# QueensGambit/CrazyAra

Hardware: AMD Instinct MI355X
Metric: nn_evals_per_sec (higher is better)
Workload: dtype f16x3; 1 GPU; crazyhouse RISEv2 19-block (34x8x8 planes -> 5184 policy + value), batch=256, inputs resident in HBM, random-init seeded weights; batch=256, parallelism=replicas x1, precision=float16x3

## Files before the change

### crazyara_amd/csrc/nn/precision.cpp

```cpp
#include <cstdlib>
#include <stdexcept>

#include "rise_net.h"

namespace cra {

namespace {
constexpr bool kX3ValueHeadOneLaunch = true;
}

RiseNet::DevSwitches::DevSwitches() {
    if (const char* e = getenv("CRA_X3_CONV_DEV")) conv_dev = atoi(e);
    device_graph = getenv("CRA_DEVICE_GRAPH") != nullptr;
    lane_graph = getenv("CRA_LANE_GRAPH") != nullptr;
    lane_no_graph = getenv("CRA_LANE_NO_GRAPH") != nullptr;
    predict_copy = getenv("CRA_PREDICT_COPY") != nullptr;
    predict_zero_copy = getenv("CRA_PREDICT_ZERO_COPY") != nullptr;
    if (const char* e = getenv("CRA_LANE_LAUNCHES")) lane_launches = e[0];
    lane_sync = getenv("CRA_LANE_SYNC") != nullptr;
    if (const char* e = getenv("CRA_X3_TOWER")) x3_symmetric = e[0] == 's';
    if (const char* e = getenv("CRA_X3_SPLIT_DEV")) x3_split_dev = atoi(e);
    no_small_path = getenv("CRA_NO_SMALL_PATH") != nullptr;
    if (const char* e = getenv("CRA_SMALL_BATCH_CONV_SPLIT")) small_conv_split = atoi(e);
    tower_trace = getenv("CRA_TOWER_TRACE") != nullptr;
    x3_value_one_launch = kX3ValueHeadOneLaunch;
    if (const char* e = getenv("CRA_X3_VALUE_HEAD")) x3_value_one_launch = e[0] == 'o';
    value_head_debug = getenv("CRA_VALUE_HEAD_DEBUG") != nullptr;
    if (const char* e = getenv("CRA_VALUE_HEAD_LDS_PAD")) value_head_lds_pad = atoi(e);
    if (const char* e = getenv("CRA_VALUE_HEAD_VARIANT")) value_head_variant = atoi(e);
    x3_no_head_chain = getenv("CRA_X3_NO_HEAD_CHAIN") != nullptr;
    x3_no_tail = getenv("CRA_X3_NO_TAIL") != nullptr;
    x3_no_quad = getenv("CRA_X3_NO_QUAD") != nullptr;
    small_batch_heads_apart = getenv("CRA_SMALL_BATCH_HEADS_APART") != nullptr;
}

Precision parse_precision(const std::string& precision) {
    Precision v;
    std::string prec = precision;
    auto strip = [&](const std::string& tag) {
        if (prec.size() <= tag.size() || prec.compare(prec.size() - tag.size(), tag.size(), tag) != 0) return false;
        prec.resize(prec.size() - tag.size());
        return true;
    };
    if (strip("-3k")) v.one_launch = false;
    if (strip("-8w")) v.thin_waves = true;
    if (strip("-1wg")) v.board_split = false;
    if (strip("-1b")) v.boards_per_wg = 1;
    else if (strip("-2b")) v.boards_per_wg = 2;
// ... 32 lines not shown
```

### crazyara_amd/csrc/nn/rise_net.h

```cpp
#pragma once
#include <hip/hip_runtime.h>
#include <memory>
#include <string>
#include <utility>
#include <vector>

#include "board_net.h"
#include "netfile.h"

namespace cra {

uint8_t float_to_e4m3(float v);
uint8_t float_to_e5m2(float v);

struct Precision {
    enum class Mode { Float32, Float16, Float16x3, Float16p8, Fp8, Int8 };
    Mode mode = Mode::Float16;
    bool fused = true;
    bool tower = true;
    bool one_launch = true;
    bool thin_waves = false;
    bool board_split = true;
    bool wblock = false;
    bool wnet = false;
// ... 96 lines not shown
        char lane_launches = 0;
        bool lane_sync = false;
        bool x3_symmetric = false;
        int x3_split_dev = 0;
        bool no_small_path = false;
        int small_conv_split = 2;
        bool tower_trace = false;
        bool x3_value_one_launch;
        bool value_head_debug = false;
        int value_head_lds_pad = -1;
        int value_head_variant = 0;
        bool x3_no_head_chain = false;
        bool x3_no_tail = false;
        bool x3_no_quad = false;
        bool small_batch_heads_apart = false;
        DevSwitches();
    } dev_;
    float* value_head_dbg_ = nullptr;

    std::string model_file_path_;
    Precision prec_;
    std::vector<std::pair<float, float>> int8_calib_;
    static constexpr int kBoardSplitMaxBatch = 64;
    std::unique_ptr<RiseNet> small_;
    bool owns_stream_ = true;
    int stream_slot_ = -1;
    std::string precision_arg_;
    int cu_count_ = 256;
    int launches_ = 0;
    hipGraph_t graph_ = nullptr;
// ... 12 lines not shown
```

### crazyara_amd/csrc/nn/rise_net.hip

```cpp
#include "rise_net.h"

#include <cmath>
#include <cstdio>
#include <cstring>
#include <fstream>
#include <algorithm>

#include "net_streams.h"
#include "onnx_import.h"
#include "rise_net_impl.h"
#include "../chess/planes_host.h"

namespace cra {

RiseNet::RiseNet(const std::string& model_path, int device_id, int batch_size, const std::string& precision, const RiseNet* parent)
    : BoardNet(device_id), impl_(new Impl) {
    if (batch_size <= 0) throw std::invalid_argument("batch size must be positive");
    precision_arg_ = precision;
    prec_ = parse_precision(precision);
    design_.batch = batch_size;

    std::string dir, file;
    auto ends_with = [&](const char* ext) { const size_t n = strlen(ext); return model_path.size() > n && model_path.compare(model_path.size() - n, n, ext) == 0; };
    if (ends_with(".cranet") || ends_with(".onnx")) {
// ... 60 lines not shown
    const int B = n > 0 ? n : design_.batch;
    const Op& op = im.ops[i];
    auto boards = [&](ConvArgs c) {
        if (n > 0 && c.batch == design_.batch && !c.out_rows_f32) c.batch = n;
        return c;
    };
    const float* planes = io ? io->planes : d_planes_;
    float* value = io ? io->value : d_value_;
    float* probs = io ? io->probs : d_probs_;
    float* aux = (io && d_aux_) ? (io->aux ? io->aux : d_aux_) : d_aux_;
    switch (op.kind) {
        case OpKind::PlanesToAct:
            launch_planes_to_act<T>(op.x == d_planes_ ? planes : static_cast<const float*>(op.x), static_cast<T*>(op.y), B, op.C, im.cin_pad, s);
            break;
        case OpKind::Conv:
            if (prec_.x3() && dev_.conv_dev >= 0) {
                ConvArgs c = boards(op.conv);
                c.dev = dev_.conv_dev;
                if (op.from_planes) c.planes = planes;
                if (op.fused_softmax) { c.softmax_out = probs; if (!keep_logits_) c.out = nullptr; }
                launch_conv_gemm_x3(c, s);
            } else if (prec_.x3() && op.from_planes) {
                ConvArgs c = boards(op.conv);
                c.planes = planes;
                launch_conv_gemm_x3(c, s);
            } else if (prec_.x3() && op.fused_softmax) {
                ConvArgs c = boards(op.conv);
                c.softmax_out = probs;
                if (!keep_logits_) c.out = nullptr;
                launch_conv_gemm_x3(c, s);
            } else if (prec_.x3()) launch_conv_gemm_x3(boards(op.conv), s);
// ... 152 lines not shown
        case OpKind::BlockX3Split: return "block_x3_split";
        case OpKind::X3SplitFinish: return "x3_split_finish";
        case OpKind::HeadsSmall: return "heads_small";
        case OpKind::Attention: return "attention";
        case OpKind::BlockX3W: return "block_x3w";
        case OpKind::NtbX3W: return "ntb_x3w";
        case OpKind::TowerX3W: return "tower_x3w";
        case OpKind::BlockX3WSplit: return "block_x3w_split";
        case OpKind::X3WSplitFinish: return "x3w_split_finish";
    }
    return "?";
}

const char* RiseNet::op_kernel(int i) const {
    const Op& op = impl_->ops.at(i);
    return op.kind == OpKind::TowerX3 ? tower_x3_kernel_name(op.tx) : op_name(i);
}

void RiseNet::time_ops(int iters, float* ms) {
    HIP_CHECK(hipSetDevice(device_));
    hipEvent_t e0, e1;
    HIP_CHECK(hipEventCreate(&e0));
    HIP_CHECK(hipEventCreate(&e1));
    const int n = int(impl_->ops.size());
    for (int it = 0; it < iters; ++it)
        for (int i = 0; i < n; ++i) {
            HIP_CHECK(hipEventRecord(e0, stream_));
            ForwardCall call;
            if (prec_.fp16()) launch_op<half_t>(i, stream_, call); else launch_op<float>(i, stream_, call);
            HIP_CHECK(hipEventRecord(e1, stream_));
// ... 453 lines not shown
```

### crazyara_amd/csrc/nn/rise_net_build.hip

```cpp
#include <algorithm>
#include <cmath>
#include <cstring>
#include <type_traits>

#include "../chess/planes_host.h"
#include "pack.h"
#include "rise_net_impl.h"

namespace cra {

namespace {
enum class Family {
    Tower,
    X3Tower,
    X3Split,
    Fused,
    WBlock,
    WSplit,
    WTower,
    Layers,
    Transformer,
    WNtb
};
struct BlockPlan {
// ... 50 lines not shown
    void add_se(Op op, bool consumer_fused);
    void stem();
    void dense_tower();
    void dense_layer_blocks();
    void bottleneck_blocks();
    void transformer_block(size_t i);
    void transformer_block_x3w(const NtbFold& n);
    void flush_tower();
    void flush_x3_run();
    void wsplit_finish();
    void flush_wrun();
    void one_launch_head();
    void policy_head();
    void softmax();
    void value_head();
    void merge_heads_small();
    void merge_forward();
};

template <typename T> void RiseNet::Builder<T>::read_model() {
    B = net.design_.batch;
    cin = int(nf.num("nb_input_channels"));
    C = int(nf.num("channels", 256));
    const int cop_init = int(nf.num("channels_operating_init"));
    const int cexp = int(nf.num("channel_expansion"));
    cv = int(nf.num("channels_value_head", 8));
    fc = int(nf.num("value_fc_size", 256));
    cp = int(nf.num("channels_policy_head"));
    wdl = nf.num("use_wdl") != 0 && nf.num("use_plys_to_end") != 0;
    std::vector<std::string> kernels = nf.list("kernels");
// ... 837 lines not shown
    im.ops.push_back(op);
}

template <typename T> void RiseNet::Builder<T>::merge_heads_small() {
    std::vector<Op>& ops = im.ops;
    if (x3_split && ops.size() >= 2 && ops.back().kind == OpKind::ValueHead && ops[ops.size() - 2].kind == OpKind::Conv &&
        ops[ops.size() - 2].fused_softmax && heads_small_fits(ops[ops.size() - 2].conv, ops.back().vh) && !dev.small_batch_heads_apart) {
        Op vh = ops.back();
        ops.pop_back();
        Op& op = ops.back();
        op.kind = OpKind::HeadsSmall;
        op.vh = vh.vh;
    }
}

template <typename T> void RiseNet::Builder<T>::merge_forward() {
    std::vector<Op>& ops = im.ops;
    if (prec.one_launch && ops.size() == 3 && ops[0].kind == OpKind::Stem && ops[1].kind == OpKind::Tower && ops[2].kind == OpKind::Head &&
        ops[1].tw.gate_in == nullptr && ops[1].tw.pool_out == nullptr) {
        Op op;
        op.kind = OpKind::Forward;
        op.st = ops[0].st;
        op.tw = ops[1].tw;
        op.hd = ops[2].hd;
        ops.assign(1, op);
        init_forward_kernel_attributes();
    }
}

template <typename T> void RiseNet::build(const NetFile& nf) {
// ... 6 lines not shown
    if (prec_.wnet && b.wblock_ops == 0 && b.wntb_ops == 0)
        throw std::runtime_error(std::string(prec_.wtower ? "`-wtower`" : "`-wnet`") + " runs the mobile-bottleneck and transformer blocks of 128 / 192 / 224-channel nets in one launch each: no block of this model qualifies (" +
                                 std::to_string(b.C) + " channels, " + (b.dense_blocks ? "dense residual blocks" : "mobile-bottleneck blocks") +
                                 "); use the precision without the suffix");
    if (prec_.wblock && !prec_.wnet && b.wblock_ops == 0)
        throw std::runtime_error("`-wblock` runs the mobile-bottleneck blocks of 128 / 192 / 224-channel nets in one launch each: no block of this model qualifies (" +
                                 std::to_string(b.C) + " channels, " + (b.dense_blocks ? "dense residual blocks" : "mobile-bottleneck blocks") +
                                 "); use the precision without the suffix");
    if (b.head_ok) {
        b.one_launch_head();
    } else {
        b.policy_head();
        b.softmax();
        b.value_head();
        b.merge_heads_small();
    }
    init_block_kernel_attributes<T>();
    init_x3_kernel_attributes();
    init_x3_wblock_kernel_attributes();
    init_x3_wsplit_kernel_attributes();
    init_x3_wtower_kernel_attributes();
    init_x3_wntb_kernel_attributes();
    init_tower_kernel_attributes();
    init_restower_kernel_attributes();
    init_head_kernel_attributes();
    b.merge_forward();
    design_.flops_per_position = 2.0 * b.macs;
    launches_ = int(impl_->ops.size());
}

template void RiseNet::build<half_t>(const NetFile& nf);
template void RiseNet::build<float>(const NetFile& nf);

// ... 2 lines not shown
```

### crazyara_amd/csrc/nn/rise_net_impl.h

```cpp
#pragma once
#include <stdexcept>
#include <string>
#include <utility>
#include <vector>

#include "kernels.h"
#include "rise_net.h"

namespace cra {

#define HIP_CHECK(expr)                                                                                      \
    do {                                                                                                     \
        hipError_t _e = (expr);                                                                              \
        if (_e != hipSuccess)                                                                                \
            throw std::runtime_error(std::string("HIP error ") + hipGetErrorString(_e) + " at " #expr);      \
    } while (0)

enum class OpKind { PlanesToAct, Conv, Depthwise, SE, ValueHead, Softmax, Block, ValueFinal, SEGate, Tower, Head, Stem, ResTower, Forward, TowerX3, BlockX3Split, X3SplitFinish, HeadsSmall, Attention, BlockX3W, NtbX3W, BlockX3WSplit, X3WSplitFinish, TowerX3W };

struct Op {
    OpKind kind;
    ConvArgs conv{};
    bool from_planes = false;
    bool fused_softmax = false;
    const void* x = nullptr;
    void* y = nullptr;
    const float *w0 = nullptr, *w1 = nullptr, *b0 = nullptr;
    int C = 0, ks = 0, se_kind = 0;
    ValueHeadArgs vh{};
    BlockArgs blk{};
    NtbArgs ntb{};
    ValueFinalArgs vf{};
    TowerArgs tw{};
    HeadArgs hd{};
    ResTowerArgs rt{};
    StemArgs st{};
    X3TowerArgs tx{};
    X3SplitArgs xs{};
    float* xs_y = nullptr;
// ... 44 lines not shown
```

### crazyara_amd/csrc/nn/x3.hip

```cpp
#include "kernels.h"
#include "device_utils.h"
#include "value_head_body.h"
#include "x3_device.h"

#include <algorithm>
#include <cstdlib>
#include <stdexcept>
#include <type_traits>

#ifndef X3_SGB_VALU
#define X3_SGB_VALU 10
#endif

namespace cra {

namespace {

typedef int i32x4_x3 __attribute__((ext_vector_type(4)));
typedef int i32x8_x3 __attribute__((ext_vector_type(8)));
__device__ __forceinline__ uint32_t x3_high_bytes(uint32_t p01, uint32_t p23) {
    return __builtin_amdgcn_perm(p23, p01, 0x07050301u);
}
__device__ __forceinline__ void split4_b8(const float (&v)[4], half4& hi, uint32_t& h8, uint32_t& l8) {
    uint32_t h[2], l[2];
// ... 9 lines not shown
    else asm volatile("" : "+v"(c) : "v"(a), "v"(b));
}
__device__ __forceinline__ i32x8_x3 x3_cat(const half8& lo16, const half8& hi16) {
    return __builtin_shufflevector(__builtin_bit_cast(i32x4_x3, lo16), __builtin_bit_cast(i32x4_x3, hi16), 0, 1, 2, 3, 4, 5, 6, 7);
}

__device__ __forceinline__ float fmac_shr1(float acc, float x, float w) { return fmaf(w, dpp_mov<DPP_ROW_SHR1>(x), acc); }
__device__ __forceinline__ float fmac_shl1(float acc, float x, float w) { return fmaf(w, dpp_mov<DPP_ROW_SHL1>(x), acc); }

__device__ __forceinline__ void mma_x3(const half8& ah, const half8& al, const half8& bh, const half8& bl, f32x4& c) {
    c = __builtin_amdgcn_mfma_f32_16x16x32_f16(al, bh, c, 0, 0, 0);
    c = __builtin_amdgcn_mfma_f32_16x16x32_f16(ah, bl, c, 0, 0, 0);
    c = __builtin_amdgcn_mfma_f32_16x16x32_f16(ah, bh, c, 0, 0, 0);
}

constexpr int X3_KC = 128;
constexpr int X3_ROWP = X3_KC + 8;

}

template <int MT, int NW>
__device__ __forceinline__ void conv_x3_finish(const ConvArgs& a, f32x4 (&acc)[MT][4], const bool (&active)[MT], char* smem, int b, int co_tile0, float acc_scale) {
    constexpr int NTHR = 64 * NW;
    const int tid = threadIdx.x;
    const int wave = tid >> 6, lane = tid & 63;
    const int l15 = lane & 15, lg = lane >> 4;
    if (a.softmax_out) __syncthreads();
#pragma unroll
    for (int m = 0; m < MT; ++m) {
        if (!active[m]) continue;
        const int co0 = (co_tile0 + m) * 16 + lg * 4;
        float bs[4];
#pragma unroll
        for (int r = 0; r < 4; ++r) bs[r] = a.bias[co0 + r];
#pragma unroll
        for (int t = 0; t < 4; ++t) {
            const int sq = t * 16 + l15;
            float v[4];
#pragma unroll
            for (int r = 0; r < 4; ++r) v[r] = fmaf(acc[m][t][r], acc_scale, bs[r]);
            if (a.relu == 2) {
#pragma unroll
                for (int r = 0; r < 4; ++r) v[r] = fmaxf(v[r], 0.f);
            }
            if (a.resid) {
                float rv[4];
                load4<float>(reinterpret_cast<const float*>(a.resid) + (size_t(b) * kSquares + sq) * a.cout_ld + co0, rv);
#pragma unroll
                for (int r = 0; r < 4; ++r) v[r] += rv[r];
            }
            if (a.relu == 1) {
#pragma unroll
                for (int r = 0; r < 4; ++r) v[r] = fmaxf(v[r], 0.f);
            }
            if (a.out_policy_f32) {
                float* o = reinterpret_cast<float*>(a.out) + size_t(b) * a.cout_real * kSquares;
                float* lds_logits = reinterpret_cast<float*>(smem);
#pragma unroll
                for (int r = 0; r < 4; ++r)
                    if (co0 + r < a.cout_real) {
                        if (a.out) o[(co0 + r) * kSquares + sq] = v[r];
                        if (a.softmax_out) lds_logits[(co0 + r) * kSquares + sq] = v[r];
                    }
            } else if (a.out_rows_f32) {
                const int row = b * kSquares + sq;
                if (row < a.rows_valid) {
                    float* o = reinterpret_cast<float*>(a.out) + size_t(row) * a.cout_real;
#pragma unroll
                    for (int r = 0; r < 4; ++r)
                        if (co0 + r < a.cout_real) o[co0 + r] = v[r];
                }
            } else if (a.out_flat) {
                float* o = reinterpret_cast<float*>(a.out) + size_t(b) * a.flat_pitch;
#pragma unroll
                for (int r = 0; r < 4; ++r)
                    if (co0 + r < a.cout_real) o[(co0 + r) * kSquares + sq] = v[r];
            } else {
                store4<float>(reinterpret_cast<float*>(a.out) + (size_t(b) * kSquares + sq) * a.cout_ld + co0, v);
            }
        }
    }
    if (a.softmax_out) {
        __syncthreads();
        const float* in = reinterpret_cast<const float*>(smem);
        float* red = reinterpret_cast<float*>(smem) + 8192;
        const int n = a.cout_real * kSquares;
        float* out = a.softmax_out + size_t(b) * n;
        float m = -INFINITY;
        for (int i = tid; i < n; i += NTHR) m = fmaxf(m, in[i]);
#pragma unroll
        for (int off = 32; off > 0; off >>= 1) m = fmaxf(m, __shfl_xor(m, off, 64));
        if (lane == 0) red[wave] = m;
        __syncthreads();
        m = red[0];
#pragma unroll
        for (int i = 1; i < NW; ++i) m = fmaxf(m, red[i]);
        float sum = 0.f;
        for (int i = tid; i < n; i += NTHR) sum += expf(in[i] - m);
#pragma unroll
        for (int off = 32; off > 0; off >>= 1) sum += __shfl_xor(sum, off, 64);
        __syncthreads();
        if (lane == 0) red[wave] = sum;
        __syncthreads();
        sum = red[0];
#pragma unroll
        for (int i = 1; i < NW; ++i) sum += red[i];
        const float c = m + logf(sum);
        for (int i = tid; i < n; i += NTHR) out[i] = expf(in[i] - c);
    }
}

template <int KS, int MT, int NW, int NS>
__device__ __forceinline__ void conv_gemm_x3_body(const ConvArgs& a, char* smem, const int bx, const int b) {
    half_t* xh = reinterpret_cast<half_t*>(smem);
    half_t* xl = xh + 65 * X3_ROWP;
    constexpr int ROWP = X3_ROWP, KC = X3_KC, NTHR = 64 * NW;

    const int tid = threadIdx.x;
    const int wave = tid >> 6, lane = tid & 63;
    const int l15 = lane & 15, lg = lane >> 4;
    const int co_tile0 = (bx * NW + wave) * MT;
    bool active[MT];
#pragma unroll
    for (int m = 0; m < MT; ++m) active[m] = (co_tile0 + m) * 16 < a.cout_pad;
    const int x_ld = a.x_ld ? a.x_ld : a.cin;
// ... 390 lines not shown
#pragma unroll
    for (int t = 0; t < 4; ++t) acc2[0][t] = f32x4{0.f, 0.f, 0.f, 0.f};
    ConvP8Window<1> W;
    if (active[0]) conv_p8_prime<1>(W, wph, wp8, 0, nslab_ci);
    __syncthreads();
    if (active[0]) {
#pragma unroll 1
        for (int pass = 0; pass < 2; ++pass) {
            if (pass == 1) conv_p8_prime<1>(W, wph, wp8, KC, nslab_ci);
            conv_p8_pass<1>(W, ConvP8::xh_of(smem, pass), ConvP8::x8_of(smem, pass), wph, wp8, pass * KC, nslab_ci, l15, lg, acc2);
        }
    }
    conv_x3_finish<1, NW>(a, acc2, active, smem, b, wave, a.acc_scale);
}

namespace {
struct ConvX3 {
    static constexpr int KC = X3_KC, ROWP = X3_ROWP, NS = KC / 32, NSTEP = 9 * NS, D = 3;
    static constexpr size_t buf_bytes = size_t(2) * 65 * ROWP * sizeof(half_t);
    static constexpr size_t lds_bytes = 2 * buf_bytes;
    static __device__ __forceinline__ half_t* xh_of(char* smem, int buf) { return reinterpret_cast<half_t*>(smem + buf * buf_bytes); }
    static __device__ __forceinline__ half_t* xl_of(char* smem, int buf) { return xh_of(smem, buf) + 65 * ROWP; }
};
template <int MT> struct ConvX3Window { half8 wh[ConvX3::D][MT], wl[ConvX3::D][MT]; };
template <int MT>
__device__ __forceinline__ void conv_x3_wload(ConvX3Window<MT>& W, const half8* const (&wph)[MT], const half8* const (&wpl)[MT], int kc0, int nslab_ci, int st) {
    const size_t wo = size_t((st / ConvX3::NS) * nslab_ci + (kc0 >> 5) + st % ConvX3::NS) * 64;
#pragma unroll
    for (int m = 0; m < MT; ++m) { W.wh[st % ConvX3::D][m] = wph[m][wo]; W.wl[st % ConvX3::D][m] = wpl[m][wo]; }
}
template <int MT>
__device__ __forceinline__ void conv_x3_prime(ConvX3Window<MT>& W, const half8* const (&wph)[MT], const half8* const (&wpl)[MT], int kc0, int nslab_ci) {
#pragma unroll
    for (int st = 0; st < ConvX3::D; ++st) conv_x3_wload<MT>(W, wph, wpl, kc0, nslab_ci, st);
}
template <int MT>
__device__ __forceinline__ void conv_x3_pass(ConvX3Window<MT>& W, const half_t* xh, const half_t* xl, const half8* const (&wph)[MT],
                                             const half8* const (&wpl)[MT], int kc0, int nslab_ci, int l15, int lg, f32x4 (&acc)[MT][4]) {
    constexpr int ROWP = ConvX3::ROWP, NS = ConvX3::NS, NSTEP = ConvX3::NSTEP, D = ConvX3::D;
    half8 bh[2][4], bl[2][4];
    auto read_frag = [&](int st) {
        const int tap = st / NS, sl = st % NS, dy = tap / 3 - 1, dx = tap % 3 - 1;
#pragma unroll
        for (int t = 0; t < 4; ++t) {
            const int sq = t * 16 + l15;
            const int ny = (sq >> 3) + dy, nx = (sq & 7) + dx;
            const bool ok = (unsigned(ny) < 8u) && (unsigned(nx) < 8u);
            const int off = (ok ? ny * 8 + nx : 64) * ROWP + lg * 8 + sl * 32;
            bh[st & 1][t] = *reinterpret_cast<const half8*>(xh + off);
            bl[st & 1][t] = *reinterpret_cast<const half8*>(xl + off);
        }
    };
    read_frag(0);
#pragma unroll
    for (int st = 0; st < NSTEP; ++st) {
        if (st + 1 < NSTEP) read_frag(st + 1);
        __builtin_amdgcn_sched_barrier(0);
#pragma unroll
        for (int m = 0; m < MT; ++m)
#pragma unroll
            for (int t = 0; t < 4; ++t) acc[m][t] = __builtin_amdgcn_mfma_f32_16x16x32_f16(W.wl[st % D][m], bh[st & 1][t], acc[m][t], 0, 0, 0);
#pragma unroll
        for (int m = 0; m < MT; ++m)
#pragma unroll
            for (int t = 0; t < 4; ++t) acc[m][t] = __builtin_amdgcn_mfma_f32_16x16x32_f16(W.wh[st % D][m], bl[st & 1][t], acc[m][t], 0, 0, 0);
#pragma unroll
        for (int m = 0; m < MT; ++m)
#pragma unroll
            for (int t = 0; t < 4; ++t) acc[m][t] = __builtin_amdgcn_mfma_f32_16x16x32_f16(W.wh[st % D][m], bh[st & 1][t], acc[m][t], 0, 0, 0);
        if (st + D < NSTEP) conv_x3_wload<MT>(W, wph, wpl, kc0, nslab_ci, st + D);
        __builtin_amdgcn_sched_barrier(0);
    }
}
struct ConvX3Stage {
    static constexpr int NV = kSquares * (ConvX3::KC / 8) / 512;
    float pre[NV][8];
    __device__ __forceinline__ void request(const float* xb, int cin, int kc0, int tid) {
#pragma unroll
        for (int j = 0; j < NV; ++j) {
            const int i = tid + j * 512, r = i / (ConvX3::KC / 8), v = i - r * (ConvX3::KC / 8);
            load8<float>(xb + size_t(r) * cin + kc0 + v * 8, pre[j]);
        }
    }
    __device__ __forceinline__ void split_store(half_t* xh, half_t* xl, int tid) {
#pragma unroll
        for (int j = 0; j < NV; ++j) {
            const int i = tid + j * 512, r = i / (ConvX3::KC / 8), v = i - r * (ConvX3::KC / 8);
            half8 h, l;
            split8(pre[j], h, l);
            *reinterpret_cast<half8*>(xh + r * ConvX3::ROWP + v * 8) = h;
            *reinterpret_cast<half8*>(xl + r * ConvX3::ROWP + v * 8) = l;
        }
    }
};
}

__global__ __launch_bounds__(512) void conv3x3_x3_chain_kernel(const ConvArgs a) {
    extern __shared__ __attribute__((aligned(16))) char smem[];
    constexpr int KC = ConvX3::KC, ROWP = ConvX3::ROWP, NW = 8, C = 256;
    const int b = blockIdx.y;
    const int tid = threadIdx.x;
    const int wave = tid >> 6, lane = tid & 63;
    const int l15 = lane & 15, lg = lane >> 4;
    const float* xb = reinterpret_cast<const float*>(a.x) + size_t(b) * kSquares * C;
    constexpr int nslab_ci = C >> 5, nslab = 9 * nslab_ci;
    {
        const half8 *wph[2], *wpl[2];
#pragma unroll
        for (int m = 0; m < 2; ++m) {
            wph[m] = reinterpret_cast<const half8*>(a.pre_wpk) + size_t(wave * 2 + m) * nslab * 64 + lane;
// ... 1386 lines not shown
```

Measured before the change: 361,700 evals/s.

## Fuse float16x3 policy conv chain and value head into one kernel

Adds a conv3x3_x3_heads_kernel that runs the policy-head conv chain with fused softmax and the value head for each board in a single launch. Two waves compute the value head from a board copy staged in LDS, in parallel with the policy conv waves. The builder merges the trailing policy Conv op and the ValueHead op into this kernel for x3 (non-p8) at large batch unless an environment switch opts out. The aim is to remove one kernel launch and the value head's second read of the tower output, at the cost of more LDS per workgroup and a value-head path that only covers one fixed head shape.

Result: faster. 367,900 evals/s, median of 6 (+1.7%).

```diff
diff --git a/crazyara_amd/csrc/nn/precision.cpp b/crazyara_amd/csrc/nn/precision.cpp
--- a/crazyara_amd/csrc/nn/precision.cpp
+++ b/crazyara_amd/csrc/nn/precision.cpp
@@ -32,6 +32,8 @@
     x3_no_tail = getenv("CRA_X3_NO_TAIL") != nullptr;
     x3_no_quad = getenv("CRA_X3_NO_QUAD") != nullptr;
     small_batch_heads_apart = getenv("CRA_SMALL_BATCH_HEADS_APART") != nullptr;
+    if (const char* e = getenv("CRA_X3_HEADS_APART")) x3_heads_apart = e[0] != '0' && e[0] != 0;
+    value_head_env = getenv("CRA_X3_VALUE_HEAD") != nullptr || getenv("CRA_VALUE_HEAD_VARIANT") != nullptr;
 }
 
 Precision parse_precision(const std::string& precision) {
diff --git a/crazyara_amd/csrc/nn/rise_net.h b/crazyara_amd/csrc/nn/rise_net.h
--- a/crazyara_amd/csrc/nn/rise_net.h
+++ b/crazyara_amd/csrc/nn/rise_net.h
@@ -134,6 +134,8 @@
         bool x3_no_tail = false;
         bool x3_no_quad = false;
         bool small_batch_heads_apart = false;
+        bool x3_heads_apart = false;
+        bool value_head_env = false;
         DevSwitches();
     } dev_;
     float* value_head_dbg_ = nullptr;
diff --git a/crazyara_amd/csrc/nn/rise_net.hip b/crazyara_amd/csrc/nn/rise_net.hip
--- a/crazyara_amd/csrc/nn/rise_net.hip
+++ b/crazyara_amd/csrc/nn/rise_net.hip
@@ -98,7 +98,17 @@
             launch_planes_to_act<T>(op.x == d_planes_ ? planes : static_cast<const float*>(op.x), static_cast<T*>(op.y), B, op.C, im.cin_pad, s);
             break;
         case OpKind::Conv:
-            if (prec_.x3() && dev_.conv_dev >= 0) {
+            if (op.heads_x3) {
+                HeadsX3Args h;
+                h.conv = boards(op.conv);
+                h.conv.softmax_out = probs;
+                if (!keep_logits_) h.conv.out = nullptr;
+                h.vh = op.vh;
+                h.vh.value = value;
+                h.vh.aux = aux;
+                h.vh.batch = h.conv.batch;
+                launch_heads_x3(h, s);
+            } else if (prec_.x3() && dev_.conv_dev >= 0) {
                 ConvArgs c = boards(op.conv);
                 c.dev = dev_.conv_dev;
                 if (op.from_planes) c.planes = planes;
@@ -281,6 +291,8 @@
 
 const char* RiseNet::op_kernel(int i) const {
     const Op& op = impl_->ops.at(i);
+    if (op.kind == OpKind::Conv && op.heads_x3) return kHeadsX3KernelName;
+    if (op.kind == OpKind::Conv && prec_.x3() && !op.conv.p8 && op.conv.pre_wpk) return "conv3x3_x3_chain_kernel";
     return op.kind == OpKind::TowerX3 ? tower_x3_kernel_name(op.tx) : op_name(i);
 }
 
diff --git a/crazyara_amd/csrc/nn/rise_net_build.hip b/crazyara_amd/csrc/nn/rise_net_build.hip
--- a/crazyara_amd/csrc/nn/rise_net_build.hip
+++ b/crazyara_amd/csrc/nn/rise_net_build.hip
@@ -88,6 +88,7 @@
     void policy_head();
     void softmax();
     void value_head();
+    void merge_heads_x3();
     void merge_heads_small();
     void merge_forward();
 };
@@ -955,6 +956,18 @@
     }
 }
 
+template <typename T> void RiseNet::Builder<T>::merge_heads_x3() {
+    std::vector<Op>& ops = im.ops;
+    if (!(prec.x3() && !prec.p8() && B > RiseNet::kBoardSplitMaxBatch && !dev.x3_heads_apart && !dev.value_head_env && dev.conv_dev < 0)) return;
+    if (ops.size() < 2 || ops.back().kind != OpKind::ValueHead || ops[ops.size() - 2].kind != OpKind::Conv) return;
+    const Op& pol = ops[ops.size() - 2];
+    if (!pol.fused_softmax || pol.from_planes || !heads_x3_fits(pol.conv, ops.back().vh) || pol.conv.batch != ops.back().vh.batch) return;
+    const ValueHeadArgs vh = ops.back().vh;
+    ops.pop_back();
+    ops.back().heads_x3 = true;
+    ops.back().vh = vh;
+}
+
 template <typename T> void RiseNet::Builder<T>::merge_forward() {
     std::vector<Op>& ops = im.ops;
     if (prec.one_launch && ops.size() == 3 && ops[0].kind == OpKind::Stem && ops[1].kind == OpKind::Tower && ops[2].kind == OpKind::Head &&
@@ -991,9 +1004,11 @@
         b.softmax();
         b.value_head();
         b.merge_heads_small();
+        b.merge_heads_x3();
     }
     init_block_kernel_attributes<T>();
     init_x3_kernel_attributes();
+    init_x3_heads_kernel_attributes();
     init_x3_wblock_kernel_attributes();
     init_x3_wsplit_kernel_attributes();
     init_x3_wtower_kernel_attributes();
diff --git a/crazyara_amd/csrc/nn/rise_net_impl.h b/crazyara_amd/csrc/nn/rise_net_impl.h
--- a/crazyara_amd/csrc/nn/rise_net_impl.h
+++ b/crazyara_amd/csrc/nn/rise_net_impl.h
@@ -6,6 +6,7 @@
 
 #include "kernels.h"
 #include "rise_net.h"
+#include "x3_heads.h"
 
 namespace cra {
 
@@ -23,6 +24,7 @@
     ConvArgs conv{};
     bool from_planes = false;
     bool fused_softmax = false;
+    bool heads_x3 = false;
     const void* x = nullptr;
     void* y = nullptr;
     const float *w0 = nullptr, *w1 = nullptr, *b0 = nullptr;
diff --git a/crazyara_amd/csrc/nn/x3.hip b/crazyara_amd/csrc/nn/x3.hip
--- a/crazyara_amd/csrc/nn/x3.hip
+++ b/crazyara_amd/csrc/nn/x3.hip
@@ -2,6 +2,7 @@
 #include "device_utils.h"
 #include "value_head_body.h"
 #include "x3_device.h"
+#include "x3_conv_device.h"
 
 #include <algorithm>
 #include <cstdlib>
@@ -47,101 +48,8 @@
     c = __builtin_amdgcn_mfma_f32_16x16x32_f16(ah, bh, c, 0, 0, 0);
 }
 
-constexpr int X3_KC = 128;
-constexpr int X3_ROWP = X3_KC + 8;
-
-}
-
-template <int MT, int NW>
-__device__ __forceinline__ void conv_x3_finish(const ConvArgs& a, f32x4 (&acc)[MT][4], const bool (&active)[MT], char* smem, int b, int co_tile0, float acc_scale) {
-    constexpr int NTHR = 64 * NW;
-    const int tid = threadIdx.x;
-    const int wave = tid >> 6, lane = tid & 63;
-    const int l15 = lane & 15, lg = lane >> 4;
-    if (a.softmax_out) __syncthreads();
-#pragma unroll
-    for (int m = 0; m < MT; ++m) {
-        if (!active[m]) continue;
-        const int co0 = (co_tile0 + m) * 16 + lg * 4;
-        float bs[4];
-#pragma unroll
-        for (int r = 0; r < 4; ++r) bs[r] = a.bias[co0 + r];
-#pragma unroll
-        for (int t = 0; t < 4; ++t) {
-            const int sq = t * 16 + l15;
-            float v[4];
-#pragma unroll
-            for (int r = 0; r < 4; ++r) v[r] = fmaf(acc[m][t][r], acc_scale, bs[r]);
-            if (a.relu == 2) {
-#pragma unroll
-                for (int r = 0; r < 4; ++r) v[r] = fmaxf(v[r], 0.f);
-            }
-            if (a.resid) {
-                float rv[4];
-                load4<float>(reinterpret_cast<const float*>(a.resid) + (size_t(b) * kSquares + sq) * a.cout_ld + co0, rv);
-#pragma unroll
-                for (int r = 0; r < 4; ++r) v[r] += rv[r];
-            }
-            if (a.relu == 1) {
-#pragma unroll
-                for (int r = 0; r < 4; ++r) v[r] = fmaxf(v[r], 0.f);
-            }
-            if (a.out_policy_f32) {
-                float* o = reinterpret_cast<float*>(a.out) + size_t(b) * a.cout_real * kSquares;
-                float* lds_logits = reinterpret_cast<float*>(smem);
-#pragma unroll
-                for (int r = 0; r < 4; ++r)
-                    if (co0 + r < a.cout_real) {
-                        if (a.out) o[(co0 + r) * kSquares + sq] = v[r];
-                        if (a.softmax_out) lds_logits[(co0 + r) * kSquares + sq] = v[r];
-                    }
-            } else if (a.out_rows_f32) {
-                const int row = b * kSquares + sq;
-                if (row < a.rows_valid) {
-                    float* o = reinterpret_cast<float*>(a.out) + size_t(row) * a.cout_real;
-#pragma unroll
-                    for (int r = 0; r < 4; ++r)
-                        if (co0 + r < a.cout_real) o[co0 + r] = v[r];
-                }
-            } else if (a.out_flat) {
-                float* o = reinterpret_cast<float*>(a.out) + size_t(b) * a.flat_pitch;
-#pragma unroll
-                for (int r = 0; r < 4; ++r)
-                    if (co0 + r < a.cout_real) o[(co0 + r) * kSquares + sq] = v[r];
-            } else {
-                store4<float>(reinterpret_cast<float*>(a.out) + (size_t(b) * kSquares + sq) * a.cout_ld + co0, v);
-            }
-        }
-    }
-    if (a.softmax_out) {
-        __syncthreads();
-        const float* in = reinterpret_cast<const float*>(smem);
-        float* red = reinterpret_cast<float*>(smem) + 8192;
-        const int n = a.cout_real * kSquares;
-        float* out = a.softmax_out + size_t(b) * n;
-        float m = -INFINITY;
-        for (int i = tid; i < n; i += NTHR) m = fmaxf(m, in[i]);
-#pragma unroll
-        for (int off = 32; off > 0; off >>= 1) m = fmaxf(m, __shfl_xor(m, off, 64));
-        if (lane == 0) red[wave] = m;
-        __syncthreads();
-        m = red[0];
-#pragma unroll
-        for (int i = 1; i < NW; ++i) m = fmaxf(m, red[i]);
-        float sum = 0.f;
-        for (int i = tid; i < n; i += NTHR) sum += expf(in[i] - m);
-#pragma unroll
-        for (int off = 32; off > 0; off >>= 1) sum += __shfl_xor(sum, off, 64);
-        __syncthreads();
-        if (lane == 0) red[wave] = sum;
-        __syncthreads();
-        sum = red[0];
-#pragma unroll
-        for (int i = 1; i < NW; ++i) sum += red[i];
-        const float c = m + logf(sum);
-        for (int i = tid; i < n; i += NTHR) out[i] = expf(in[i] - c);
-    }
-}
+}
+
 
 template <int KS, int MT, int NW, int NS>
 __device__ __forceinline__ void conv_gemm_x3_body(const ConvArgs& a, char* smem, const int bx, const int b) {
@@ -562,86 +470,6 @@
     conv_x3_finish<1, NW>(a, acc2, active, smem, b, wave, a.acc_scale);
 }
 
-namespace {
-struct ConvX3 {
-    static constexpr int KC = X3_KC, ROWP = X3_ROWP, NS = KC / 32, NSTEP = 9 * NS, D = 3;
-    static constexpr size_t buf_bytes = size_t(2) * 65 * ROWP * sizeof(half_t);
-    static constexpr size_t lds_bytes = 2 * buf_bytes;
-    static __device__ __forceinline__ half_t* xh_of(char* smem, int buf) { return reinterpret_cast<half_t*>(smem + buf * buf_bytes); }
-    static __device__ __forceinline__ half_t* xl_of(char* smem, int buf) { return xh_of(smem, buf) + 65 * ROWP; }
-};
-template <int MT> struct ConvX3Window { half8 wh[ConvX3::D][MT], wl[ConvX3::D][MT]; };
-template <int MT>
-__device__ __forceinline__ void conv_x3_wload(ConvX3Window<MT>& W, const half8* const (&wph)[MT], const half8* const (&wpl)[MT], int kc0, int nslab_ci, int st) {
-    const size_t wo = size_t((st / ConvX3::NS) * nslab_ci + (kc0 >> 5) + st % ConvX3::NS) * 64;
-#pragma unroll
-    for (int m = 0; m < MT; ++m) { W.wh[st % ConvX3::D][m] = wph[m][wo]; W.wl[st % ConvX3::D][m] = wpl[m][wo]; }
-}
-template <int MT>
-__device__ __forceinline__ void conv_x3_prime(ConvX3Window<MT>& W, const half8* const (&wph)[MT], const half8* const (&wpl)[MT], int kc0, int nslab_ci) {
-#pragma unroll
-    for (int st = 0; st < ConvX3::D; ++st) conv_x3_wload<MT>(W, wph, wpl, kc0, nslab_ci, st);
-}
-template <int MT>
-__device__ __forceinline__ void conv_x3_pass(ConvX3Window<MT>& W, const half_t* xh, const half_t* xl, const half8* const (&wph)[MT],
-                                             const half8* const (&wpl)[MT], int kc0, int nslab_ci, int l15, int lg, f32x4 (&acc)[MT][4]) {
-    constexpr int ROWP = ConvX3::ROWP, NS = ConvX3::NS, NSTEP = ConvX3::NSTEP, D = ConvX3::D;
-    half8 bh[2][4], bl[2][4];
-    auto read_frag = [&](int st) {
-        const int tap = st / NS, sl = st % NS, dy = tap / 3 - 1, dx = tap % 3 - 1;
-#pragma unroll
-        for (int t = 0; t < 4; ++t) {
-            const int sq = t * 16 + l15;
-            const int ny = (sq >> 3) + dy, nx = (sq & 7) + dx;
-            const bool ok = (unsigned(ny) < 8u) && (unsigned(nx) < 8u);
-            const int off = (ok ? ny * 8 + nx : 64) * ROWP + lg * 8 + sl * 32;
-            bh[st & 1][t] = *reinterpret_cast<const half8*>(xh + off);
-            bl[st & 1][t] = *reinterpret_cast<const half8*>(xl + off);
-        }
-    };
-    read_frag(0);
-#pragma unroll
-    for (int st = 0; st < NSTEP; ++st) {
-        if (st + 1 < NSTEP) read_frag(st + 1);
-        __builtin_amdgcn_sched_barrier(0);
-#pragma unroll
-        for (int m = 0; m < MT; ++m)
-#pragma unroll
-            for (int t = 0; t < 4; ++t) acc[m][t] = __builtin_amdgcn_mfma_f32_16x16x32_f16(W.wl[st % D][m], bh[st & 1][t], acc[m][t], 0, 0, 0);
-#pragma unroll
-        for (int m = 0; m < MT; ++m)
-#pragma unroll
-            for (int t = 0; t < 4; ++t) acc[m][t] = __builtin_amdgcn_mfma_f32_16x16x32_f16(W.wh[st % D][m], bl[st & 1][t], acc[m][t], 0, 0, 0);
-#pragma unroll
-        for (int m = 0; m < MT; ++m)
-#pragma unroll
-            for (int t = 0; t < 4; ++t) acc[m][t] = __builtin_amdgcn_mfma_f32_16x16x32_f16(W.wh[st % D][m], bh[st & 1][t], acc[m][t], 0, 0, 0);
-        if (st + D < NSTEP) conv_x3_wload<MT>(W, wph, wpl, kc0, nslab_ci, st + D);
-        __builtin_amdgcn_sched_barrier(0);
-    }
-}
-struct ConvX3Stage {
-    static constexpr int NV = kSquares * (ConvX3::KC / 8) / 512;
-    float pre[NV][8];
-    __device__ __forceinline__ void request(const float* xb, int cin, int kc0, int tid) {
-#pragma unroll
-        for (int j = 0; j < NV; ++j) {
-            const int i = tid + j * 512, r = i / (ConvX3::KC / 8), v = i - r * (ConvX3::KC / 8);
-            load8<float>(xb + size_t(r) * cin + kc0 + v * 8, pre[j]);
-        }
-    }
-    __device__ __forceinline__ void split_store(half_t* xh, half_t* xl, int tid) {
-#pragma unroll
-        for (int j = 0; j < NV; ++j) {
-            const int i = tid + j * 512, r = i / (ConvX3::KC / 8), v = i - r * (ConvX3::KC / 8);
-            half8 h, l;
-            split8(pre[j], h, l);
-            *reinterpret_cast<half8*>(xh + r * ConvX3::ROWP + v * 8) = h;
-            *reinterpret_cast<half8*>(xl + r * ConvX3::ROWP + v * 8) = l;
-        }
-    }
-};
-}
 
 __global__ __launch_bounds__(512) void conv3x3_x3_chain_kernel(const ConvArgs a) {
     extern __shared__ __attribute__((aligned(16))) char smem[];
diff --git a/crazyara_amd/csrc/nn/x3_conv_device.h b/crazyara_amd/csrc/nn/x3_conv_device.h
--- /dev/null
+++ b/crazyara_amd/csrc/nn/x3_conv_device.h
@@ -0,0 +1,185 @@
+#pragma once
+#include "kernels.h"
+#include "device_utils.h"
+#include "x3_device.h"
+
+namespace cra {
+
+namespace {
+constexpr int X3_KC = 128;
+constexpr int X3_ROWP = X3_KC + 8;
+}
+
+template <int MT, int NW>
+__device__ __forceinline__ void conv_x3_finish(const ConvArgs& a, f32x4 (&acc)[MT][4], const bool (&active)[MT], char* smem, int b, int co_tile0, float acc_scale) {
+    constexpr int NTHR = 64 * NW;
+    const int tid = threadIdx.x;
+    const int wave = tid >> 6, lane = tid & 63;
+    const int l15 = lane & 15, lg = lane >> 4;
+    if (a.softmax_out) __syncthreads();
+#pragma unroll
+    for (int m = 0; m < MT; ++m) {
+        if (!active[m]) continue;
+        const int co0 = (co_tile0 + m) * 16 + lg * 4;
+        float bs[4];
+#pragma unroll
+        for (int r = 0; r < 4; ++r) bs[r] = a.bias[co0 + r];
+#pragma unroll
+        for (int t = 0; t < 4; ++t) {
+            const int sq = t * 16 + l15;
+            float v[4];
+#pragma unroll
+            for (int r = 0; r < 4; ++r) v[r] = fmaf(acc[m][t][r], acc_scale, bs[r]);
+            if (a.relu == 2) {
+#pragma unroll
+                for (int r = 0; r < 4; ++r) v[r] = fmaxf(v[r], 0.f);
+            }
+            if (a.resid) {
+                float rv[4];
+                load4<float>(reinterpret_cast<const float*>(a.resid) + (size_t(b) * kSquares + sq) * a.cout_ld + co0, rv);
+#pragma unroll
+                for (int r = 0; r < 4; ++r) v[r] += rv[r];
+            }
+            if (a.relu == 1) {
+#pragma unroll
+                for (int r = 0; r < 4; ++r) v[r] = fmaxf(v[r], 0.f);
+            }
+            if (a.out_policy_f32) {
+                float* o = reinterpret_cast<float*>(a.out) + size_t(b) * a.cout_real * kSquares;
+                float* lds_logits = reinterpret_cast<float*>(smem);
+#pragma unroll
+                for (int r = 0; r < 4; ++r)
+                    if (co0 + r < a.cout_real) {
+                        if (a.out) o[(co0 + r) * kSquares + sq] = v[r];
+                        if (a.softmax_out) lds_logits[(co0 + r) * kSquares + sq] = v[r];
+                    }
+            } else if (a.out_rows_f32) {
+                const int row = b * kSquares + sq;
+                if (row < a.rows_valid) {
+                    float* o = reinterpret_cast<float*>(a.out) + size_t(row) * a.cout_real;
+#pragma unroll
+                    for (int r = 0; r < 4; ++r)
+                        if (co0 + r < a.cout_real) o[co0 + r] = v[r];
+                }
+            } else if (a.out_flat) {
+                float* o = reinterpret_cast<float*>(a.out) + size_t(b) * a.flat_pitch;
+#pragma unroll
+                for (int r = 0; r < 4; ++r)
+                    if (co0 + r < a.cout_real) o[(co0 + r) * kSquares + sq] = v[r];
+            } else {
+                store4<float>(reinterpret_cast<float*>(a.out) + (size_t(b) * kSquares + sq) * a.cout_ld + co0, v);
+            }
+        }
+    }
+    if (a.softmax_out) {
+        __syncthreads();
+        const float* in = reinterpret_cast<const float*>(smem);
+        float* red = reinterpret_cast<float*>(smem) + 8192;
+        const int n = a.cout_real * kSquares;
+        float* out = a.softmax_out + size_t(b) * n;
+        float m = -INFINITY;
+        for (int i = tid; i < n; i += NTHR) m = fmaxf(m, in[i]);
+#pragma unroll
+        for (int off = 32; off > 0; off >>= 1) m = fmaxf(m, __shfl_xor(m, off, 64));
+        if (lane == 0) red[wave] = m;
+        __syncthreads();
+        m = red[0];
+#pragma unroll
+        for (int i = 1; i < NW; ++i) m = fmaxf(m, red[i]);
+        float sum = 0.f;
+        for (int i = tid; i < n; i += NTHR) sum += expf(in[i] - m);
+#pragma unroll
+        for (int off = 32; off > 0; off >>= 1) sum += __shfl_xor(sum, off, 64);
+        __syncthreads();
+        if (lane == 0) red[wave] = sum;
+        __syncthreads();
+        sum = red[0];
+#pragma unroll
+        for (int i = 1; i < NW; ++i) sum += red[i];
+        const float c = m + logf(sum);
+        for (int i = tid; i < n; i += NTHR) out[i] = expf(in[i] - c);
+    }
+}
+
+namespace {
+struct ConvX3 {
+    static constexpr int KC = X3_KC, ROWP = X3_ROWP, NS = KC / 32, NSTEP = 9 * NS, D = 3;
+    static constexpr size_t buf_bytes = size_t(2) * 65 * ROWP * sizeof(half_t);
+    static constexpr size_t lds_bytes = 2 * buf_bytes;
+    static __device__ __forceinline__ half_t* xh_of(char* smem, int buf) { return reinterpret_cast<half_t*>(smem + buf * buf_bytes); }
+    static __device__ __forceinline__ half_t* xl_of(char* smem, int buf) { return xh_of(smem, buf) + 65 * ROWP; }
+};
+template <int MT> struct ConvX3Window { half8 wh[ConvX3::D][MT], wl[ConvX3::D][MT]; };
+template <int MT>
+__device__ __forceinline__ void conv_x3_wload(ConvX3Window<MT>& W, const half8* const (&wph)[MT], const half8* const (&wpl)[MT], int kc0, int nslab_ci, int st) {
+    const size_t wo = size_t((st / ConvX3::NS) * nslab_ci + (kc0 >> 5) + st % ConvX3::NS) * 64;
+#pragma unroll
+    for (int m = 0; m < MT; ++m) { W.wh[st % ConvX3::D][m] = wph[m][wo]; W.wl[st % ConvX3::D][m] = wpl[m][wo]; }
+}
+template <int MT>
+__device__ __forceinline__ void conv_x3_prime(ConvX3Window<MT>& W, const half8* const (&wph)[MT], const half8* const (&wpl)[MT], int kc0, int nslab_ci) {
+#pragma unroll
+    for (int st = 0; st < ConvX3::D; ++st) conv_x3_wload<MT>(W, wph, wpl, kc0, nslab_ci, st);
+}
+template <int MT>
+__device__ __forceinline__ void conv_x3_pass(ConvX3Window<MT>& W, const half_t* xh, const half_t* xl, const half8* const (&wph)[MT],
+                                             const half8* const (&wpl)[MT], int kc0, int nslab_ci, int l15, int lg, f32x4 (&acc)[MT][4]) {
+    constexpr int ROWP = ConvX3::ROWP, NS = ConvX3::NS, NSTEP = ConvX3::NSTEP, D = ConvX3::D;
+    half8 bh[2][4], bl[2][4];
+    auto read_frag = [&](int st) {
+        const int tap = st / NS, sl = st % NS, dy = tap / 3 - 1, dx = tap % 3 - 1;
+#pragma unroll
+        for (int t = 0; t < 4; ++t) {
+            const int sq = t * 16 + l15;
+            const int ny = (sq >> 3) + dy, nx = (sq & 7) + dx;
+            const bool ok = (unsigned(ny) < 8u) && (unsigned(nx) < 8u);
+            const int off = (ok ? ny * 8 + nx : 64) * ROWP + lg * 8 + sl * 32;
+            bh[st & 1][t] = *reinterpret_cast<const half8*>(xh + off);
+            bl[st & 1][t] = *reinterpret_cast<const half8*>(xl + off);
+        }
+    };
+    read_frag(0);
+#pragma unroll
+    for (int st = 0; st < NSTEP; ++st) {
+        if (st + 1 < NSTEP) read_frag(st + 1);
+        __builtin_amdgcn_sched_barrier(0);
+#pragma unroll
+        for (int m = 0; m < MT; ++m)
+#pragma unroll
+            for (int t = 0; t < 4; ++t) acc[m][t] = __builtin_amdgcn_mfma_f32_16x16x32_f16(W.wl[st % D][m], bh[st & 1][t], acc[m][t], 0, 0, 0);
+#pragma unroll
+        for (int m = 0; m < MT; ++m)
+#pragma unroll
+            for (int t = 0; t < 4; ++t) acc[m][t] = __builtin_amdgcn_mfma_f32_16x16x32_f16(W.wh[st % D][m], bl[st & 1][t], acc[m][t], 0, 0, 0);
+#pragma unroll
+        for (int m = 0; m < MT; ++m)
+#pragma unroll
+            for (int t = 0; t < 4; ++t) acc[m][t] = __builtin_amdgcn_mfma_f32_16x16x32_f16(W.wh[st % D][m], bh[st & 1][t], acc[m][t], 0, 0, 0);
+        if (st + D < NSTEP) conv_x3_wload<MT>(W, wph, wpl, kc0, nslab_ci, st + D);
+        __builtin_amdgcn_sched_barrier(0);
+    }
+}
+struct ConvX3Stage {
+    static constexpr int NV = kSquares * (ConvX3::KC / 8) / 512;
+    float pre[NV][8];
+    __device__ __forceinline__ void request(const float* xb, int cin, int kc0, int tid) {
+#pragma unroll
+        for (int j = 0; j < NV; ++j) {
+            const int i = tid + j * 512, r = i / (ConvX3::KC / 8), v = i - r * (ConvX3::KC / 8);
+            load8<float>(xb + size_t(r) * cin + kc0 + v * 8, pre[j]);
+        }
+    }
+    __device__ __forceinline__ void split_store(half_t* xh, half_t* xl, int tid) {
+#pragma unroll
+        for (int j = 0; j < NV; ++j) {
+            const int i = tid + j * 512, r = i / (ConvX3::KC / 8), v = i - r * (ConvX3::KC / 8);
+            half8 h, l;
+            split8(pre[j], h, l);
+            *reinterpret_cast<half8*>(xh + r * ConvX3::ROWP + v * 8) = h;
+            *reinterpret_cast<half8*>(xl + r * ConvX3::ROWP + v * 8) = l;
+        }
+    }
+};
+}
+
+}
diff --git a/crazyara_amd/csrc/nn/x3_heads.cpp b/crazyara_amd/csrc/nn/x3_heads.cpp
--- /dev/null
+++ b/crazyara_amd/csrc/nn/x3_heads.cpp
@@ -0,0 +1,211 @@
+#include "x3_heads.h"
+#include "device_utils.h"
+#include "value_head_body.h"
+#include "x3_device.h"
+#include "x3_conv_device.h"
+
+#include <stdexcept>
+
+namespace cra {
+
+namespace {
+struct HeadsX3 {
+    static constexpr int C = 256, CV = 8, FC = 256, XP = C + 4;
+    static constexpr size_t xs_off = ConvX3::lds_bytes;
+    static constexpr size_t ws_off = xs_off + size_t(kSquares) * XP * sizeof(float);
+    static constexpr size_t flat_off = ws_off + size_t(CV) * C * sizeof(float);
+    static constexpr size_t part_off = flat_off + size_t(CV) * kSquares * sizeof(float);
+    static constexpr size_t red_off = part_off + size_t(8) * FC * sizeof(float);
+    static constexpr size_t lds_bytes = red_off + 8 * sizeof(float);
+};
+static_assert(HeadsX3::xs_off % 16 == 0 && HeadsX3::lds_bytes <= 160 * 1024, "LDS budget");
+
+__device__ __forceinline__ void heads_x3_store_board(const ConvX3Stage& stage, float* xs, int kc0, int tid) {
+#pragma unroll
+    for (int j = 0; j < ConvX3Stage::NV; ++j) {
+        const int i = tid + j * 512, r = i / (ConvX3::KC / 8), v = i - r * (ConvX3::KC / 8);
+        float* p = xs + r * HeadsX3::XP + kc0 + v * 8;
+        *reinterpret_cast<f32x4*>(p) = f32x4{stage.pre[j][0], stage.pre[j][1], stage.pre[j][2], stage.pre[j][3]};
+        *reinterpret_cast<f32x4*>(p + 4) = f32x4{stage.pre[j][4], stage.pre[j][5], stage.pre[j][6], stage.pre[j][7]};
+    }
+}
+
+__device__ __forceinline__ void heads_x3_value_wave(const ValueHeadArgs& v, const float* xs, const float* ws, float* s_flat, float* s_part, int vw, int lane) {
+    constexpr int C = HeadsX3::C, XP = HeadsX3::XP, FC = HeadsX3::FC;
+    const float* wt = v.w1t + size_t(vw) * 256 * FC + 4 * lane;
+    f32x4 w[32];
+#pragma unroll
+    for (int j = 0; j < 32; ++j) w[j] = *reinterpret_cast<const f32x4*>(wt + size_t(j) * FC);
+    __builtin_amdgcn_sched_barrier(0);
+    {
+        float acc[4] = {0.f, 0.f, 0.f, 0.f};
+        const float* xr = xs + lane * XP;
+        const float* wr = ws + vw * 4 * C;
+#pragma unroll 2
+        for (int c = 0; c < C; c += 4) {
+            const f32x4 xv = *reinterpret_cast<const f32x4*>(xr + c);
+#pragma unroll
+            for (int k = 0; k < 4; ++k) {
+                const f32x4 wv = *reinterpret_cast<const f32x4*>(wr + k * C + c);
+                acc[k] = fmaf(wv[0], xv[0], acc[k]);
+                acc[k] = fmaf(wv[1], xv[1], acc[k]);
+                acc[k] = fmaf(wv[2], xv[2], acc[k]);
+                acc[k] = fmaf(wv[3], xv[3], acc[k]);
+            }
+        }
+#pragma unroll
+        for (int k = 0; k < 4; ++k) s_flat[(vw * 4 + k) * kSquares + lane] = fmaxf(acc[k] + v.bconv[vw * 4 + k], 0.f);
+    }
+    __builtin_amdgcn_fence(__ATOMIC_RELEASE, "wavefront");
+    __builtin_amdgcn_wave_barrier();
+    __builtin_amdgcn_fence(__ATOMIC_ACQUIRE, "wavefront");
+    const float* fl = s_flat + vw * 256;
+    f32x4 h = {0.f, 0.f, 0.f, 0.f};
+#pragma unroll
+    for (int bt = 0; bt < 8; ++bt) {
+        if ((bt & 1) == 0) h = f32x4{0.f, 0.f, 0.f, 0.f};
+#pragma unroll
+        for (int q = 0; q < 8; ++q) {
+            const f32x4 f = *reinterpret_cast<const f32x4*>(fl + bt * 32 + 4 * q);
+#pragma unroll
+            for (int e = 0; e < 4; ++e) {
+                const int j = 4 * q + e;
+                float h0 = h[0], h1 = h[1], h2 = h[2], h3 = h[3];
+                const float w0 = w[j][0], w1 = w[j][1], w2 = w[j][2], w3 = w[j][3], fe = f[e];
+                asm volatile("v_fmac_f32 %0, %4, %8\n\tv_fmac_f32 %1, %5, %8\n\tv_fmac_f32 %2, %6, %8\n\tv_fmac_f32 %3, %7, %8"
+                             : "+v"(h0), "+v"(h1), "+v"(h2), "+v"(h3) : "v"(w0), "v"(w1), "v"(w2), "v"(w3), "v"(fe));
+                h = f32x4{h0, h1, h2, h3};
+                if (bt + 1 < 8) w[j] = *reinterpret_cast<const f32x4*>(wt + size_t((bt + 1) * 32 + j) * FC);
+                __builtin_amdgcn_sched_barrier(0);
+            }
+        }
+        if (bt & 1) *reinterpret_cast<f32x4*>(s_part + (vw * 4 + bt / 2) * FC + 4 * lane) = h;
+    }
+}
+}
+
+__global__ __launch_bounds__(512) void conv3x3_x3_heads_kernel(const HeadsX3Args args) {
+    extern __shared__ __attribute__((aligned(16))) char smem[];
+    const ConvArgs& a = args.conv;
+    const ValueHeadArgs& vh = args.vh;
+    constexpr int KC = ConvX3::KC, ROWP = ConvX3::ROWP, NW = 8, C = 256;
+    const int b = blockIdx.y;
+    const int tid = threadIdx.x;
+    const int wave = tid >> 6, lane = tid & 63;
+    const int l15 = lane & 15, lg = lane >> 4;
+    const float* xb = reinterpret_cast<const float*>(a.x) + size_t(b) * kSquares * C;
+    constexpr int nslab_ci = C >> 5, nslab = 9 * nslab_ci;
+    float* xs = reinterpret_cast<float*>(smem + HeadsX3::xs_off);
+    float* ws = reinterpret_cast<float*>(smem + HeadsX3::ws_off);
+    float* s_flat = reinterpret_cast<float*>(smem + HeadsX3::flat_off);
+    float* s_part = reinterpret_cast<float*>(smem + HeadsX3::part_off);
+    float* s_red = reinterpret_cast<float*>(smem + HeadsX3::red_off);
+    {
+        const half8 *wph[2], *wpl[2];
+#pragma unroll
+        for (int m = 0; m < 2; ++m) {
+            wph[m] = reinterpret_cast<const half8*>(a.pre_wpk) + size_t(wave * 2 + m) * nslab * 64 + lane;
+            wpl[m] = reinterpret_cast<const half8*>(a.pre_wpk_lo) + size_t(wave * 2 + m) * nslab * 64 + lane;
+        }
+        f32x4 acc[2][4];
+#pragma unroll
+        for (int m = 0; m < 2; ++m)
+#pragma unroll
+            for (int t = 0; t < 4; ++t) acc[m][t] = f32x4{0.f, 0.f, 0.f, 0.f};
+        for (int i = tid; i < 4 * ROWP; i += 512) {
+            const int tile = i / ROWP, c = i - tile * ROWP;
+            (tile & 1 ? ConvX3::xl_of(smem, tile >> 1) : ConvX3::xh_of(smem, tile >> 1))[64 * ROWP + c] = half_t(0.f);
+        }
+        const f32x4 wcv = *reinterpret_cast<const f32x4*>(vh.wconv + tid * 4);
+        ConvX3Stage stage;
+        stage.request(xb, C, 0, tid);
+        stage.split_store(ConvX3::xh_of(smem, 0), ConvX3::xl_of(smem, 0), tid);
+        heads_x3_store_board(stage, xs, 0, tid);
+        *reinterpret_cast<f32x4*>(ws + tid * 4) = wcv;
+#pragma unroll 1
+        for (int pass = 0; pass < 2; ++pass) {
+            const int kc0 = pass * KC;
+            ConvX3Window<2> W;
+            conv_x3_prime<2>(W, wph, wpl, kc0, nslab_ci);
+            __syncthreads();
+            if (pass == 0) stage.request(xb, C, KC, tid);
+            conv_x3_pass<2>(W, ConvX3::xh_of(smem, pass), ConvX3::xl_of(smem, pass), wph, wpl, kc0, nslab_ci, l15, lg, acc);
+            if (pass == 0) {
+                stage.split_store(ConvX3::xh_of(smem, 1), ConvX3::xl_of(smem, 1), tid);
+                heads_x3_store_board(stage, xs, KC, tid);
+            }
+        }
+        __syncthreads();
+#pragma unroll
+        for (int m = 0; m < 2; ++m) {
+            const int c0 = (wave * 2 + m) * 16 + lg * 4;
+            const f32x4 bs = *reinterpret_cast<const f32x4*>(a.pre_bias + c0);
+            half_t* xh = ConvX3::xh_of(smem, c0 >> 7);
+            half_t* xl = ConvX3::xl_of(smem, c0 >> 7);
+#pragma unroll
+            for (int t = 0; t < 4; ++t) {
+                const int sq = t * 16 + l15;
+                float v[4];
+#pragma unroll
+                for (int r = 0; r < 4; ++r) v[r] = fmaxf(fmaf(acc[m][t][r], 1.f, bs[r]), 0.f);
+                half4 h, l;
+                split4(v, h, l);
+                *reinterpret_cast<half4*>(xh + sq * ROWP + (c0 & 127)) = h;
+                *reinterpret_cast<half4*>(xl + sq * ROWP + (c0 & 127)) = l;
+            }
+        }
+    }
+    bool active[1] = {wave * 16 < a.cout_pad};
+    const half8 *wph[1], *wpl[1];
+    wph[0] = reinterpret_cast<const half8*>(a.wpk) + size_t(active[0] ? wave : 0) * nslab * 64 + lane;
+    wpl[0] = reinterpret_cast<const half8*>(a.wpk_lo) + size_t(active[0] ? wave : 0) * nslab * 64 + lane;
+    f32x4 acc2[1][4];
+#pragma unroll
+    for (int t = 0; t < 4; ++t) acc2[0][t] = f32x4{0.f, 0.f, 0.f, 0.f};
+    ConvX3Window<1> W;
+    if (active[0]) conv_x3_prime<1>(W, wph, wpl, 0, nslab_ci);
+    float b1v = 0.f, w2v = 0.f;
+    if (tid < HeadsX3::FC) { b1v = vh.b1[tid]; w2v = vh.w2[tid]; }
+    __syncthreads();
+    const int wave_u = __builtin_amdgcn_readfirstlane(wave);
+    if (wave_u >= 6) {
+        heads_x3_value_wave(vh, xs, ws, s_flat, s_part, wave_u - 6, lane);
+    } else if (active[0]) {
+#pragma unroll 1
+        for (int pass = 0; pass < 2; ++pass) {
+            if (pass == 1) conv_x3_prime<1>(W, wph, wpl, KC, nslab_ci);
+            conv_x3_pass<1>(W, ConvX3::xh_of(smem, pass), ConvX3::xl_of(smem, pass), wph, wpl, pass * KC, nslab_ci, l15, lg, acc2);
+        }
+    }
+    __syncthreads();
+    {
+        float part = 0.f;
+        if (tid < HeadsX3::FC) {
+            constexpr int FC = HeadsX3::FC;
+            const int t = tid;
+            float ps = (s_part[t] + s_part[FC + t]) + (s_part[2 * FC + t] + s_part[3 * FC + t]);
+            ps += (s_part[4 * FC + t] + s_part[5 * FC + t]) + (s_part[6 * FC + t] + s_part[7 * FC + t]);
+            const float h = b1v + ps;
+            part = fmaf(w2v, fmaxf(h, 0.f), part);
+        }
+        const float tot = block_sum<512>(part, s_red);
+        if (tid == 0) vh.value[b] = tanhf(tot + vh.b2);
+    }
+    conv_x3_finish<1, NW>(a, acc2, active, smem, b, wave, 1.f);
+}
+
+bool heads_x3_fits(const ConvArgs& c, const ValueHeadArgs& v) {
+    return c.pre_wpk && !c.p8 && c.ks == 3 && c.cin == HeadsX3::C && c.cout_pad <= 96 && !c.resid && !c.planes && !c.out_rows_f32 && c.out_policy_f32 &&
+           !c.x_ld && c.dev == 0 && !v.wwdl && !v.dbg && v.variant == 0 && v.lds_pad < 0 && v.cv == HeadsX3::CV && v.fc == HeadsX3::FC && v.C == HeadsX3::C &&
+           v.x == c.x && v.w1t && v.b1 && v.w2;
+}
+void init_x3_heads_kernel_attributes() {
+    (void)hipFuncSetAttribute(reinterpret_cast<const void*>(&conv3x3_x3_heads_kernel), hipFuncAttributeMaxDynamicSharedMemorySize, int(HeadsX3::lds_bytes));
+}
+void launch_heads_x3(const HeadsX3Args& a, hipStream_t s) {
+    if (!heads_x3_fits(a.conv, a.vh) || a.conv.batch != a.vh.batch)
+        throw std::invalid_argument("conv3x3_x3_heads_kernel: the float16x3 policy chain with at most 96 padded couts and the plain value head (8 channels, 256 FC outputs) on the same boards");
+    hipLaunchKernelGGL(conv3x3_x3_heads_kernel, dim3(1, a.conv.batch), dim3(512), HeadsX3::lds_bytes, s, a);
+}
+
+}
diff --git a/crazyara_amd/csrc/nn/x3_heads.h b/crazyara_amd/csrc/nn/x3_heads.h
--- /dev/null
+++ b/crazyara_amd/csrc/nn/x3_heads.h
@@ -0,0 +1,15 @@
+#pragma once
+#include "kernels.h"
+
+namespace cra {
+
+struct HeadsX3Args {
+    ConvArgs conv;
+    ValueHeadArgs vh;
+};
+bool heads_x3_fits(const ConvArgs& c, const ValueHeadArgs& v);
+void launch_heads_x3(const HeadsX3Args& a, hipStream_t s);
+void init_x3_heads_kernel_attributes();
+constexpr const char* kHeadsX3KernelName = "conv3x3_x3_heads_kernel";
+
+}
```
